# openai/Video-Pre-Training

Measured on AMD Instinct MI355X. Metric: frames/sec (fwd) [+ bc_step.ms_per_step], 2x policy, 128x128x3 seq=128, higher is better.
Workload: dtype bf16; 1 GPU; foundation-model-2x policy forward (IMPALA CNN + 4-layer banded transformer + heads), batch=64 seq=128 uint8 128x128x3 frames per GPU, KV memory carried, random-init weights; global_batch=64, seq_len=128, parallelism=dp1 replicas (no collective in forward; BC step: gradient all-reduce)

## Files before the change

include/vpt_hip.h:

```cpp
#ifndef VPT_HIP_H
#define VPT_HIP_H
#include <stdint.h>

#ifdef __cplusplus
extern "C" {
#endif

const char* vpt_version(void);
#define VPT_HIP_ABI 5
int vpt_abi_version(void);
const char* vpt_operand_format(void);
const char* vpt_last_error(void);

long vpt_conv3x3_packed_elems(int Cout, int Cin);
long vpt_conv3x3_table_floats(int Cout);
long vpt_linear_packed_elems(int N, int K);
long vpt_conv_first_packed_elems(int Cout);
long vpt_conv3d_t5_packed_elems(int O);
int vpt_pack_conv_first(const float* weight, const float* bias, void* wfrag, int Cout, void* stream);
int vpt_pack_conv3d_t5(const float* weight, const float* bias, void* wfrag, float* bias_padded, int O, void* stream);
int vpt_chw_to_blocked(const float* src, float* dst, int64_t rows, int C, int H, int W, void* stream);

enum { VPT_WS_CONV3X3_WGRAD = 1, VPT_WS_CONV_BACKWARD_PREPARE = 2, VPT_WS_LINEAR_SPLITK = 3, VPT_WS_LAYERNORM_BACKWARD = 4, VPT_WS_COLUMN_SUM = 5,
       VPT_WS_ATTENTION_BACKWARD_DKV = 6, VPT_WS_ATTENTION_BACKWARD_DBND = 7, VPT_WS_FRAME_AFFINE_BACKWARD = 8, VPT_WS_CONV_FIRST_BACKWARD = 9 };
// ... 48 lines not shown

int vpt_linear_wgrad(const void* dy, const void* x, float* dw, int M, int N, int K, int ldy, int ldx, int ldw, int accumulate, void* stream);

int vpt_dense_fold_epilogue(const float* part, int splitk, const double* stats, int count, const float* sg, const float* sb, float* out,
                            int M, int N, void* stream);

int vpt_linear_splitk_epilogue(const float* part, int splitk, const float* bias, const float* res, float* out_f32, void* out_bf16,
                               int M, int N, int ldr, int ldc, int ldcb, int relu, const void* mask, int ldm, void* stream);

int vpt_layernorm_linear_forward(const float* x, const float* ln_gain, const float* ln_bias, int relu_in, float* ln_out_f32,
                                 const void* wpk, const float* bias, const float* res, float* out_f32, void* out_bf16,
                                 int M, int N, int K, int ldr, int ldc, int ldcb, int relu, void* stream);

int vpt_layernorm_forward(const float* x, const float* gain, const float* bias, float* out_f32, void* out_bf16,
                          int M, int D, int relu_in, void* stream);

int vpt_masked_attention_forward(const float* qkvr, const float* kmem, const float* vmem, const uint8_t* memvalid,
                                 const float* b_nd, void* out, int B, int t, int heads, int hid, int ld,
                                 int maxlen, int causal, void* stream);

int vpt_kv_memory_update(const float* qkvr, const float* kmem, const float* vmem, float* kout, float* vout,
                         int B, int t, int hid, int ld, int maxlen, void* stream);

int vpt_masked_attention_step(const float* qkvr, const float* kmem, const float* vmem, const uint8_t* state_mask, const uint8_t* first,
                              const float* b_nd, void* out, float* kout, float* vout, uint8_t* mask_out,
                              int B, int heads, int hid, int ld, int maxlen, void* stream);

int vpt_masked_attention_step_inplace(const float* qkvr, float* kmem, float* vmem, uint8_t* state_mask, const uint8_t* first,
                                      const float* b_nd, void* out, int* done_counter, int B, int heads, int hid, int ld, int maxlen, void* stream);

int vpt_act_epilogue(const int64_t* action_buttons, const int64_t* action_camera, const float* logp_buttons, const float* logp_camera,
                     const float* logits, int ld, int value_col, float scale, float shift, int64_t* keep, uint8_t* nan_flag, uint64_t* rng_state,
                     int B, void* stream);

int vpt_log_softmax_forward(const float* logits, float* out, int M, int ld, int col0, int n, float temperature,
                            void* stream);

int vpt_action_head_forward(const float* logits, const uint8_t* mask, const float* noise, const uint64_t* rng_state, uint32_t rng_stream,
                            float* out, int64_t* action, float* action_logp, int M, int ld, int col0, int n, float temperature, void* stream);
int vpt_uniform_noise(const uint64_t* rng_state, uint32_t rng_stream, float* out, int M, int n, void* stream);

int vpt_adam_step(float* param, const float* grad, float* exp_avg, float* exp_avg_sq, uint64_t n, int step,
                  float lr, float beta1, float beta2, float eps, float weight_decay, float grad_scale, void* stream);

int vpt_adam_step_multi(const void* table, int ntensors, int64_t total_blocks, int step, float lr, float beta1, float beta2,
                        float eps, float weight_decay, float grad_scale, const int32_t* skip_flag, void* stream);
// ... 73 lines not shown
```

video-pre-training_amd/_native.py:

```python
import ctypes
import os

_HERE = os.path.dirname(os.path.abspath(__file__))
_LIB_PATH = os.environ.get("VPT_HIP_LIB") or os.path.join(_HERE, "libvpt_hip.so")
_LIB_PATHS = {"bf16": _LIB_PATH, "fp16": os.path.join(_HERE, "libvpt_hip_f16.so")}
_libs = {}

ABI_VERSION = 5

_P = ctypes.c_void_p
_I = ctypes.c_int
_F = ctypes.c_float
_L = ctypes.c_long
_D = ctypes.c_double

SIGNATURES = {
    "vpt_conv_first_forward": [_P, _P, _P, _P, _P, _P, _I, _I, _I, _I, _P],
    "vpt_conv3d_t5_forward": [_P, _P, _P, _P, _P, _I, _I, _I, _I, _I, _P],
    "vpt_pack_conv3x3": [_P, _P, _P, _P, _P, _P, _I, _I, _P],
    "vpt_pack_linear": [_P, _P, _I, _I, _I, _I, _I, _P],
    "vpt_pack_conv_first": [_P, _P, _P, _I, _P],
    "vpt_pack_conv3d_t5": [_P, _P, _P, _P, _I, _P],
    "vpt_chw_to_blocked": [_P, _P, ctypes.c_int64, _I, _I, _I, _P],
    "vpt_conv3x3_forward": [_P, _P, _P, _P, _P, _P, _P, _P, _I, _I, _I, _I, _I, _P],
    "vpt_conv3x3_forward_tiled": [_P, _P, _P, _P, _P, _P, _P, _P, _I, _I, _I, _I, _I, _I, _P],
    "vpt_conv3x3_pool_forward": [_P, _P, _P, _P, _P, _P, _P, _P, _P, _P, _I, _I, _I, _I, _I, _I, _P],
    "vpt_conv3x3_forward_folded": [_P] * 12 + [_I, _I, _I, _I, _I, _P],
    "vpt_channel_stats": [_P, _P, _I, _I, _I, _P],
    "vpt_nfold_coef": [_P] * 12 + [_I, _I, _I, _I, _P],
    "vpt_maxpool_forward": [_P, _P, _P, _P, _I, _I, _I, _I, _P],
    "vpt_frame_affine_forward": [_P, _P, _P, _P, _P, _P, _I, _I, _I, _I, _P],
    "vpt_linear_forward": [_P, _P, _P, _P, _P, _P, _I, _I, _I, _I, _I, _I, _I, _I, _I, _P, _I, _P],
    "vpt_linear_forward_tiled": [_P, _P, _P, _P, _P, _P, _I, _I, _I, _I, _I, _I, _I, _I, _I, _P, _I, _I, _P],
    "vpt_linear_wgrad": [_P, _P, _P, _I, _I, _I, _I, _I, _I, _I, _P],
    "vpt_dense_fold_epilogue": [_P, _I, _P, _I, _P, _P, _P, _I, _I, _P],
    "vpt_linear_splitk_epilogue": [_P, _I, _P, _P, _P, _P, _I, _I, _I, _I, _I, _I, _P, _I, _P],
    "vpt_layernorm_forward": [_P, _P, _P, _P, _P, _I, _I, _I, _P],
    "vpt_masked_attention_forward": [_P, _P, _P, _P, _P, _P, _I, _I, _I, _I, _I, _I, _I, _P],
    "vpt_kv_memory_update": [_P, _P, _P, _P, _P, _I, _I, _I, _I, _I, _P],
    "vpt_log_softmax_forward": [_P, _P, _I, _I, _I, _I, _F, _P],
    "vpt_action_head_forward": [_P, _P, _P, _P, ctypes.c_uint32, _P, _P, _P, _I, _I, _I, _I, _F, _P],
    "vpt_uniform_noise": [_P, ctypes.c_uint32, _P, _I, _I, _P],
    "vpt_conv_backward_prepare": [_P] * 14 + [_I, _I, _I, _I, _I, _P],
    "vpt_conv3x3_dgrad": [_P, _P, _P, _P, _P, _P, _I, _I, _I, _I, _I, _P],
    "vpt_conv3x3_pool_argmax_forward": [_P, _P, _P, _P, _P, _P, _P, _P, _P, _I, _I, _I, _I, _I, _I, _P],
    "vpt_conv_backward_prepare_pooled": [_P] * 15 + [_I, _I, _I, _I, _I, _P],
    "vpt_conv3x3_dgrad_gated": [_P, _P, _P, _P, _P, _I, _P, _P, _I, _I, _I, _I, _I, _P],
    "vpt_conv_backward_reduce": [_P] * 10 + [_I, _I, _I, _I, _I, _P],
    "vpt_conv_first_backward": [_P, _P, _P, _P, _P, _P, _I, _I, _I, _I, _P],
    "vpt_conv_first_backward_nfold": [_P, _P, _P, _P, _P, _P, _P, _P, _P, _I, _I, _I, _I, _P],
    "vpt_conv3x3_wgrad": [_P, _P, _P, _P, _I, _I, _I, _I, _I, _P],
    "vpt_conv3x3_wgrad_scratch_floats": [_I, _I, _I],
    "vpt_camera_discretize": [_P, _P, _L, _D, _D, _D, _I, _P],
    "vpt_camera_undiscretize": [_P, _P, _L, _D, _D, _D, _I, _P],
    "vpt_action_from_factored": [_P, _P, _P, _P, _L, _I, _P],
    "vpt_action_to_factored": [_P, _P, _P, _P, _L, _I, _P],
    "vpt_maxpool_backward": [_P, _P, _P, _P, _I, _I, _I, _I, _P],
    "vpt_frame_affine_backward": [_P, _P, _P, _P, _P, _P, _P, _P, _P, _P, _I, _I, _I, _I, _I, _P],
    "vpt_bc_nll_backward": [_P, _P, _P, _P, _P, _I, _I, _I, _I, _F, _P],
    "vpt_heads_logprob_backward": [_P, _P, _P, _P, _P, _P, _P, _P, _I, _I, _I, _I, _F, _F, _P],
    "vpt_layernorm_backward": [_P, _P, _P, _P, _P, _P, _P, _P, _I, _I, _I, _P],
    "vpt_gate_cast": [_P, _P, _P, _I, _I, _I, _I, _I, _P],
# ... 73 lines not shown
```

video-pre-training_amd/csrc/vpt_capi.hip:

```cpp
#include "../../include/vpt_hip.h"
#include "vpt_kernels.h"
#include "vpt_common.h"
#include <stdio.h>
#include <math.h>

static thread_local char g_err[256] = "ok";

static int fail(int code, const char* what) {
  snprintf(g_err, sizeof(g_err), "%s (code %d, hip: %s)", what, code, hipGetErrorString(hipPeekAtLastError()));
  return code;
}
#define CHECK_LAUNCH(expr, name) do { int rc_ = (expr); if (rc_ != 0) return fail(rc_, name); return 0; } while (0)

__global__ __launch_bounds__(256) void vpt_poison_lds_kernel(int words, unsigned pattern) {
  extern __shared__ unsigned poison_lds_[];
  volatile unsigned* l = poison_lds_;
  for (int i = threadIdx.x; i < words; i += 256) l[i] = pattern;
  __syncthreads();
  for (int k = 0; k < 16; ++k) __builtin_amdgcn_s_sleep(127);
}

extern "C" {

const char* vpt_version(void) { return "vpt_hip 0.5 gfx950"; }
// ... 368 lines not shown
  a.A = nullptr; a.wpk = nullptr; a.bias = bias; a.res = res; a.out_f32 = out_f32; a.out_bf16 = (vpt_op16*)out_bf16;
  a.M = M; a.N = N; a.K = 0; a.lda = 0; a.ldr = ldr; a.ldc = ldc; a.ldcb = ldcb; a.relu = relu; a.splitk = splitk; a.atomic_out = 0;
  a.mask = (const vpt_op16*)mask; a.ldm = ldm;
  CHECK_LAUNCH(vpt_splitk_epilogue_launch(part, splitk, &a, (hipStream_t)stream), "vpt_linear_splitk_epilogue");
}

int vpt_layernorm_forward(const float* x, const float* gain, const float* bias, float* out_f32, void* out_bf16,
                          int M, int D, int relu_in, void* stream) {
  VptLayerNormArgs a = {};
  a.x = x; a.gain = gain; a.bias = bias; a.out_f32 = out_f32; a.out_bf16 = (vpt_op16*)out_bf16;
  a.M = M; a.D = D; a.relu_in = relu_in;
  CHECK_LAUNCH(vpt_layernorm_launch(&a, (hipStream_t)stream), "vpt_layernorm_forward");
}

int vpt_masked_attention_forward(const float* qkvr, const float* kmem, const float* vmem, const uint8_t* memvalid,
                                 const float* b_nd, void* out, int B, int t, int heads, int hid, int ld,
                                 int maxlen, int causal, void* stream) {
  VptAttnArgs a = {};
  a.qkvr = qkvr; a.kmem = kmem; a.vmem = vmem; a.memvalid = memvalid; a.b_nd = b_nd; a.out = (vpt_op16*)out;
  a.B = B; a.t = t; a.heads = heads; a.hid = hid; a.ld = ld; a.maxlen = maxlen; a.causal = causal;
  CHECK_LAUNCH(vpt_attn_launch(&a, (hipStream_t)stream), "vpt_masked_attention_forward");
}

int vpt_masked_attention_step(const float* qkvr, const float* kmem, const float* vmem, const uint8_t* state_mask, const uint8_t* first,
                              const float* b_nd, void* out, float* kout, float* vout, uint8_t* mask_out,
                              int B, int heads, int hid, int ld, int maxlen, void* stream) {
  VptAttnArgs a = {};
  a.qkvr = qkvr; a.kmem = kmem; a.vmem = vmem; a.memvalid = nullptr; a.b_nd = b_nd; a.out = (vpt_op16*)out;
  a.B = B; a.t = 1; a.heads = heads; a.hid = hid; a.ld = ld; a.maxlen = maxlen; a.causal = 1;
  CHECK_LAUNCH(vpt_attn_step_launch(&a, state_mask, first, mask_out, kout, vout, nullptr, (hipStream_t)stream), "vpt_masked_attention_step");
}

int vpt_masked_attention_step_inplace(const float* qkvr, float* kmem, float* vmem, uint8_t* state_mask, const uint8_t* first,
                                      const float* b_nd, void* out, int* done_counter, int B, int heads, int hid, int ld, int maxlen, void* stream) {
  if (!done_counter) return fail(-1, "vpt_masked_attention_step_inplace: done_counter ([B] ints, zero before the first launch) is required");
  VptAttnArgs a = {};
  a.qkvr = qkvr; a.kmem = kmem; a.vmem = vmem; a.memvalid = nullptr; a.b_nd = b_nd; a.out = (vpt_op16*)out;
  a.B = B; a.t = 1; a.heads = heads; a.hid = hid; a.ld = ld; a.maxlen = maxlen; a.causal = 1;
  CHECK_LAUNCH(vpt_attn_step_launch(&a, state_mask, first, state_mask, kmem, vmem, done_counter, (hipStream_t)stream), "vpt_masked_attention_step_inplace");
}

int vpt_act_epilogue(const int64_t* action_buttons, const int64_t* action_camera, const float* logp_buttons, const float* logp_camera,
                     const float* logits, int ld, int value_col, float scale, float shift, int64_t* keep, uint8_t* nan_flag, uint64_t* rng_state,
                     int B, void* stream) {
  CHECK_LAUNCH(vpt_act_epilogue_launch(action_buttons, action_camera, logp_buttons, logp_camera, logits, ld, value_col, scale, shift, keep, nan_flag,
                                       rng_state, B, (hipStream_t)stream), "vpt_act_epilogue");
// ... 149 lines not shown
```

video-pre-training_amd/csrc/vpt_kernels.h:

```cpp
#pragma once
#include <hip/hip_runtime.h>
#include <stdint.h>

#ifdef VPT_OPERAND_F16
typedef _Float16 vpt_op16;
#else
typedef __bf16 vpt_op16;
#endif

struct VptConv3x3Args {
  const vpt_op16* x;
  const vpt_op16* wpk;
  const float* edge_sa;
  const float* edge_sg;
  const double* stats_in;
  const vpt_op16* res;
  vpt_op16* y;
  double* stats_out;
  int frames, H, W, Cin, Cout, CoutPad, NT;
  double inv_count_in;
  int tiling;
  int ablate;
  long long* trace;
  const float* kk_frame;
// ... 364 lines not shown
int vpt_colsum_launch(const VptColsumArgs* a, hipStream_t s);
int vpt_clip_launch(const VptClipArgs* a, hipStream_t s);
int vpt_attn_step_launch(const VptAttnArgs* a, const uint8_t* state_mask, const uint8_t* first, uint8_t* mask_out, float* kout, float* vout, int* done, hipStream_t s);
int vpt_act_epilogue_launch(const int64_t* act_b, const int64_t* act_c, const float* lp_b, const float* lp_c, const float* logits, int ld, int vcol,
                            float scale, float shift, int64_t* keep, uint8_t* nan_flag, uint64_t* rng_state, int B, hipStream_t s);
int vpt_uniform_noise_launch(const uint64_t* rng_state, uint32_t rng_stream, float* out, int M, int n, hipStream_t s);
int vpt_attn_bwd_launch(const VptAttnBwdArgs* a, hipStream_t s);
long vpt_attn_bwd_dkv_floats(int B, int t, int hid);
long vpt_attn_bwd_dbnd_floats(int B, int t, int heads, int maxlen);
long vpt_colsum_partial_floats(int M, int N);
long vpt_slab_sum_scratch_floats(int rows, int cols);
int vpt_slab_sum_launch(const float* slab, int rows, int cols, long ld, float* out_a, int split, float* out_b, int accumulate, float* scratch, hipStream_t s);
int vpt_conv3x3_launch(const VptConv3x3Args* a, hipStream_t s);
int vpt_pool_seam_launch(const VptPoolSeamArgs* a, hipStream_t s);
int vpt_channel_stats_launch(const VptChannelStatsArgs* a, hipStream_t s);
int vpt_nfold_coef_launch(const VptNfoldCoefArgs* a, hipStream_t s);
int vpt_conv_first_launch(const VptConvFirstArgs* a, hipStream_t s);
int vpt_conv3d_launch(const VptConv3dArgs* a, hipStream_t s);
int vpt_pool_launch(const VptPoolArgs* a, hipStream_t s);
int vpt_affine_launch(const VptAffineArgs* a, hipStream_t s);
int vpt_gemm_launch(const VptGemmArgs* a, hipStream_t s);
int vpt_layernorm_launch(const VptLayerNormArgs* a, hipStream_t s);
int vpt_attn_launch(const VptAttnArgs* a, hipStream_t s);
int vpt_kv_update_launch(const VptKvUpdateArgs* a, hipStream_t s);
int vpt_logsoftmax_launch(const VptLogSoftmaxArgs* a, hipStream_t s);
}
```

video-pre-training_amd/csrc/vpt_transformer.hip:

```cpp
#include "vpt_common.h"
#include "vpt_kernels.h"

__global__ __launch_bounds__(256) void vpt_layernorm_kernel(VptLayerNormArgs a) {
  const int lane = threadIdx.x & 63;
  const int row = blockIdx.x * 4 + (threadIdx.x >> 6);
  if (row >= a.M) return;
  const float* x = a.x + (size_t)row * a.D;
  const int n4 = a.D >> 2;
  float s = 0.f;
  for (int i = lane; i < n4; i += 64) {
    f32x4 v = *(const f32x4*)(x + 4 * i);
    if (a.relu_in) { v.x = fmaxf(v.x, 0.f); v.y = fmaxf(v.y, 0.f); v.z = fmaxf(v.z, 0.f); v.w = fmaxf(v.w, 0.f); }
    s += (v.x + v.y) + (v.z + v.w);
  }
  const float mean = wave_sum(s) / (float)a.D;
  float ss = 0.f;
  for (int i = lane; i < n4; i += 64) {
    f32x4 v = *(const f32x4*)(x + 4 * i);
    if (a.relu_in) { v.x = fmaxf(v.x, 0.f); v.y = fmaxf(v.y, 0.f); v.z = fmaxf(v.z, 0.f); v.w = fmaxf(v.w, 0.f); }
    const float d0 = v.x - mean, d1 = v.y - mean, d2 = v.z - mean, d3 = v.w - mean;
    ss += (d0 * d0 + d1 * d1) + (d2 * d2 + d3 * d3);
  }
  const float rstd = rsqrtf(wave_sum(ss) / (float)a.D + VPT_NORM_EPS);
  for (int i = lane; i < n4; i += 64) {
// ... 10 lines not shown
      u32x2 p = {pack_op16x2(y.x, y.y), pack_op16x2(y.z, y.w)};
      *(u32x2*)(a.out_bf16 + (size_t)row * a.D + 4 * i) = p;
    }
  }
}

extern "C" int vpt_layernorm_launch(const VptLayerNormArgs* a, hipStream_t stream) {
  if (a->M <= 0 || (a->D & 3)) return -1;
  hipLaunchKernelGGL(vpt_layernorm_kernel, dim3((a->M + 3) >> 2), dim3(256), 0, stream, *a);
  return hipGetLastError() == hipSuccess ? 0 : -3;
}

#define ATT_DH 128
#define ATT_QT 32
#define ATT_NK 160
#define ATT_RS (ATT_DH + 4)
#define ATT_SS 164
#define ATT_S_OFF 0
#define ATT_R_OFF (ATT_S_OFF + ATT_QT * ATT_SS)
#define ATT_B_OFF (ATT_R_OFF + ATT_QT * 10)
#define ATT_SC_OFF (ATT_B_OFF + 10 * 129)
#define ATT_PT_OFF ((ATT_SC_OFF + ATT_QT + 3) & ~3)
#define ATT_FLOATS (ATT_PT_OFF + 4 * 16 * 64)

__global__ __launch_bounds__(256) void vpt_attn_kernel(VptAttnArgs a) {
  extern __shared__ __attribute__((aligned(16))) float sm[];
  float* Ss = sm + ATT_S_OFF;
  float* Rs = sm + ATT_R_OFF;
  float* Bs = sm + ATT_B_OFF;
  float* Sc = sm + ATT_SC_OFF;

  const int tid = threadIdx.x, lane = tid & 63, w = __builtin_amdgcn_readfirstlane(tid >> 6);
  const int b = blockIdx.y / a.heads, h = blockIdx.y - b * a.heads;
  const int q0 = blockIdx.x * ATT_QT;
  const int maxlen = a.maxlen, t = a.t, hid = a.hid;
  const size_t tok0 = (size_t)b * t;
  const int jbase = a.causal ? q0 + 1 : 0;

  for (int idx = tid; idx < ATT_QT * 10; idx += 256) {
    const int r = idx / 10, n = idx - r * 10;
    Rs[idx] = (a.causal && q0 + r < t) ? a.qkvr[(tok0 + q0 + r) * a.ld + 3 * hid + h * 10 + n] : 0.f;
  }
  for (int idx = tid; idx < 10 * maxlen; idx += 256) Bs[idx] = a.b_nd[idx];
  __syncthreads();

  const int l31 = lane & 31, hi = lane >> 5;
  auto kv_row = [&](int j, int which) -> const float* {
    if (j < maxlen) return (which == 1 ? a.kmem : a.vmem) + ((size_t)b * maxlen + j) * hid + h * ATT_DH;
    if (j - maxlen < t) return a.qkvr + (tok0 + j - maxlen) * a.ld + which * hid + h * ATT_DH;
    return nullptr;
  };
  {
    f32x16 acc, acc4;
#pragma unroll
    for (int r = 0; r < 16; ++r) { acc[r] = 0.f; acc4[r] = 0.f; }
    const f32x4 z4 = {0.f, 0.f, 0.f, 0.f};
    const float* qa = (q0 + l31 < t) ? a.qkvr + (tok0 + q0 + l31) * a.ld + h * ATT_DH + 4 * hi : nullptr;
    const float* kr = kv_row(jbase + w * 32 + l31, 1);
    const float* kr4 = kv_row(jbase + 128 + l31, 1);
    const float* kb = kr ? kr + 4 * hi : nullptr;
    const float* kb4 = kr4 ? kr4 + 4 * hi : nullptr;
#pragma unroll 8
    for (int g = 0; g < 16; ++g) {
      const f32x4 q4 = qa ? *(const f32x4*)(qa + 8 * g) : z4, k4 = kb ? *(const f32x4*)(kb + 8 * g) : z4;
      acc = __builtin_amdgcn_mfma_f32_32x32x2f32(q4.x, k4.x, acc, 0, 0, 0);
      acc = __builtin_amdgcn_mfma_f32_32x32x2f32(q4.y, k4.y, acc, 0, 0, 0);
      acc = __builtin_amdgcn_mfma_f32_32x32x2f32(q4.z, k4.z, acc, 0, 0, 0);
      acc = __builtin_amdgcn_mfma_f32_32x32x2f32(q4.w, k4.w, acc, 0, 0, 0);
    }
#pragma unroll
    for (int g4 = 0; g4 < 4; ++g4) {
      const int g = 4 * w + g4;
      const f32x4 q4 = qa ? *(const f32x4*)(qa + 8 * g) : z4, k4 = kb4 ? *(const f32x4*)(kb4 + 8 * g) : z4;
      acc4 = __builtin_amdgcn_mfma_f32_32x32x2f32(q4.x, k4.x, acc4, 0, 0, 0);
      acc4 = __builtin_amdgcn_mfma_f32_32x32x2f32(q4.y, k4.y, acc4, 0, 0, 0);
      acc4 = __builtin_amdgcn_mfma_f32_32x32x2f32(q4.z, k4.z, acc4, 0, 0, 0);
      acc4 = __builtin_amdgcn_mfma_f32_32x32x2f32(q4.w, k4.w, acc4, 0, 0, 0);
    }
    float* Pt = sm + ATT_PT_OFF;
#pragma unroll
    for (int r = 0; r < 16; ++r) Pt[(w * 16 + r) * 64 + lane] = acc4[r];
    __syncthreads();
    auto finish = [&](int kk, int r, float dot) {
      const int qi = (r & 3) + 8 * (r >> 2) + 4 * hi;
      const bool qvalid = (q0 + qi) < t;
      const int off = maxlen - 1 + qi - kk;
      const int j = jbase + kk;
      bool vis = a.causal ? (qvalid && off >= 0 && off < maxlen) : (qvalid && kk < t);
      if (vis && a.causal && j < maxlen) vis = a.memvalid[(size_t)b * maxlen + j] != 0;
      float sc = -3.0e38f;
      if (vis) {
        float rb = 0.f;
        if (a.causal) {
#pragma unroll
          for (int n = 0; n < 10; ++n) rb = fmaf(Rs[qi * 10 + n], Bs[n * maxlen + off], rb);
        }
        sc = dot * (1.0f / ATT_DH) + rb;
      }
      Ss[qi * ATT_SS + kk] = sc;
    };
#pragma unroll
    for (int r = 0; r < 16; ++r) finish(w * 32 + l31, r, acc[r]);
#pragma unroll
    for (int r4 = 0; r4 < 4; ++r4) {
      const int r = 4 * w + r4;
      const float dot = (Pt[(0 * 16 + r) * 64 + lane] + Pt[(1 * 16 + r) * 64 + lane]) + (Pt[(2 * 16 + r) * 64 + lane] + Pt[(3 * 16 + r) * 64 + lane]);
      finish(128 + l31, r, dot);
    }
  }
  __syncthreads();
  for (int r = w * 8; r < w * 8 + 8; ++r) {
    float* srow = Ss + r * ATT_SS;
    const float s0 = srow[lane], s1 = srow[lane + 64], s2 = (lane + 128 < ATT_NK) ? srow[lane + 128] : -3.0e38f;
    const float m = wave_max(fmaxf(s0, fmaxf(s1, s2)));
    const float e0 = (s0 > -1.0e38f) ? expf(s0 - m) : 0.f;
    const float e1 = (s1 > -1.0e38f) ? expf(s1 - m) : 0.f;
    const float e2 = (s2 > -1.0e38f) ? expf(s2 - m) : 0.f;
    const float tot = wave_sum(e0 + e1 + e2);
    srow[lane] = e0;
    srow[lane + 64] = e1;
    if (lane + 128 < ATT_NK) srow[lane + 128] = e2;
    if (lane == 0) Sc[r] = (tot > 0.f) ? 1.0f / tot : 0.f;
  }
  __syncthreads();

  {
    f32x16 o;
#pragma unroll
    for (int r = 0; r < 16; ++r) o[r] = 0.f;
    const float* pa = Ss + l31 * ATT_SS + 4 * hi;
    const int dcol = w * 32 + l31;
#pragma unroll 4
    for (int g = 0; g < ATT_NK / 8; ++g) {
      const f32x4 p4 = *(const f32x4*)(pa + 8 * g);
      float v[4];
#pragma unroll
      for (int e = 0; e < 4; ++e) {
        const float* r0 = kv_row(jbase + 8 * g + e, 2);
        const float* r1 = kv_row(jbase + 8 * g + 4 + e, 2);
        const float* rr = hi ? r1 : r0;
        v[e] = rr ? rr[dcol] : 0.f;
      }
      o = __builtin_amdgcn_mfma_f32_32x32x2f32(p4.x, v[0], o, 0, 0, 0);
      o = __builtin_amdgcn_mfma_f32_32x32x2f32(p4.y, v[1], o, 0, 0, 0);
      o = __builtin_amdgcn_mfma_f32_32x32x2f32(p4.z, v[2], o, 0, 0, 0);
      o = __builtin_amdgcn_mfma_f32_32x32x2f32(p4.w, v[3], o, 0, 0, 0);
    }
#pragma unroll
    for (int r = 0; r < 16; ++r) {
      const int qi = (r & 3) + 8 * (r >> 2) + 4 * hi;
      if (q0 + qi < t) a.out[(tok0 + q0 + qi) * hid + h * ATT_DH + w * 32 + l31] = (vpt_op16)(o[r] * Sc[qi]);
    }
  }
}

extern "C" int vpt_attn_launch(const VptAttnArgs* a, hipStream_t stream) {
  if (a->hid != a->heads * ATT_DH) return -1;
  if (a->causal ? (a->maxlen < 1 || a->maxlen > 129) : (a->maxlen != 0 || a->t > ATT_NK)) return -1;
  static unsigned long long optin_done = 0;
  const size_t lds = ATT_FLOATS * sizeof(float);
  if (!vpt_lds_optin((const void*)vpt_attn_kernel, (int)lds, &optin_done)) return -4;
  dim3 grid((a->t + ATT_QT - 1) / ATT_QT, a->B * a->heads);
  hipLaunchKernelGGL(vpt_attn_kernel, grid, dim3(256), lds, stream, *a);
  return hipGetLastError() == hipSuccess ? 0 : -3;
}

struct VptAttnStepExtra {
  const uint8_t* state_mask;
  const uint8_t* first;
  uint8_t* mask_out;
  float* kout;
  float* vout;
  int* done;
};

__global__ __launch_bounds__(256) void vpt_attn_step_kernel(VptAttnArgs a, VptAttnStepExtra x) {
  __shared__ float sc_[128], red_[8], part_[128];
  __shared__ int last_;
  const int tid = threadIdx.x, lane = tid & 63, w = tid >> 6;
  const int b = blockIdx.x / a.heads, h = blockIdx.x - b * a.heads;
  const int maxlen = a.maxlen, hid = a.hid;
  const float* qrow = a.qkvr + (size_t)b * a.ld;
  auto kv_row = [&](int j, int which) -> const float* {
    if (j < maxlen) return (which == 1 ? a.kmem : a.vmem) + ((size_t)b * maxlen + j) * hid + h * ATT_DH;
    return qrow + which * hid + h * ATT_DH;
  };
// ... 94 lines not shown
  const int h4 = a.hid >> 2;
  const int c4 = (int)(idx % h4);
  const size_t rs = idx / h4;
  const int s = (int)(rs % a.maxlen);
  const int b = (int)(rs / a.maxlen);
  const int src = s + a.t;
  const float* mem = which ? a.vmem : a.kmem;
  float* out = which ? a.vout : a.kout;
  f32x4 v;
  if (src < a.maxlen) v = *(const f32x4*)(mem + ((size_t)b * a.maxlen + src) * a.hid + c4 * 4);
  else v = *(const f32x4*)(a.qkvr + ((size_t)b * a.t + (src - a.maxlen)) * a.ld + (which ? 2 : 1) * a.hid + c4 * 4);
  *(f32x4*)(out + ((size_t)b * a.maxlen + s) * a.hid + c4 * 4) = v;
}

extern "C" int vpt_kv_update_launch(const VptKvUpdateArgs* a, hipStream_t stream) {
  if (a->B <= 0 || (a->hid & 3)) return -1;
  const size_t n4 = (size_t)a->B * a->maxlen * (a->hid >> 2);
  dim3 grid((unsigned)((n4 + 255) / 256), 2);
  hipLaunchKernelGGL(vpt_kv_update_kernel, grid, dim3(256), 0, stream, *a);
  return hipGetLastError() == hipSuccess ? 0 : -3;
}

#define LSM_CAP 9
template <int NW>
__global__ __launch_bounds__(64 * NW) void vpt_logsoftmax_kernel(VptLogSoftmaxArgs a) {
  constexpr int NT = 64 * NW;
  __shared__ float red[3 * NW];
  __shared__ int redi[NW];
  const int row = blockIdx.x, tid = threadIdx.x, lane = tid & 63, w = tid >> 6;
  const float* z = a.logits + (size_t)row * a.ld + a.col0;
  const uint8_t* mk = a.mask ? a.mask + (size_t)row * a.n : nullptr;
  const float T = a.temperature;
#define SCALED(i_) ((mk && !mk[i_]) ? -100.0f : z[i_] / T)
  float c[LSM_CAP];
  float m = -3.0e38f;
#pragma unroll
  for (int k = 0; k < LSM_CAP; ++k) {
    const int i = tid + NT * k;
    c[k] = (i < a.n) ? SCALED(i) : -3.0e38f;
    m = fmaxf(m, c[k]);
  }
  for (int i = tid + NT * LSM_CAP; i < a.n; i += NT) m = fmaxf(m, SCALED(i));
  m = wave_max(m);
  if (lane == 0) red[w] = m;
  __syncthreads();
  m = red[0];
#pragma unroll
  for (int k = 1; k < NW; ++k) m = fmaxf(m, red[k]);
  float s = 0.f;
#pragma unroll
  for (int k = 0; k < LSM_CAP; ++k) s += (tid + NT * k < a.n) ? expf(c[k] - m) : 0.f;
  for (int i = tid + NT * LSM_CAP; i < a.n; i += NT) s += expf(SCALED(i) - m);
  s = wave_sum(s);
  if (lane == 0) red[NW + w] = s;
  __syncthreads();
  float tot = 0.f;
#pragma unroll
  for (int k = 0; k < NW; ++k) tot += red[NW + k];
  const float lse = m + logf(tot);
  float* o = a.out + (size_t)row * a.n;
  const float* u = a.noise ? a.noise + (size_t)row * a.n : nullptr;
  const bool gen = !u && a.rng_state != nullptr;
  uint64_t seed = 0, rstep = 0;
  if (gen) { seed = a.rng_state[0]; rstep = a.rng_state[1]; }
  float best = -3.0e38f;
  int besti = 0x7fffffff;
  auto emit = [&](int i, float sc_) __attribute__((always_inline)) {
    const float lp = sc_ - lse;
    o[i] = lp;
    if (a.action) {
      float sc = lp;
      if (u || gen) {
        float ui = u ? u[i] : vpt_philox_uniform(seed, rstep, a.rng_stream, (uint32_t)row, (uint32_t)i);
        if (ui == 1.0f) ui = 0.999f;
        sc = lp - logf(-logf(ui));
      }
      if (sc > best) { best = sc; besti = i; }
    }
  };
#pragma unroll
  for (int k = 0; k < LSM_CAP; ++k)
    if (tid + NT * k < a.n) emit(tid + NT * k, c[k]);
  for (int i = tid + NT * LSM_CAP; i < a.n; i += NT) emit(i, SCALED(i));
  if (a.action) {
#pragma unroll
    for (int off = 32; off > 0; off >>= 1) {
      const float ob = __shfl_xor(best, off, 64);
      const int oi = __shfl_xor(besti, off, 64);
      if (ob > best || (ob == best && oi < besti)) { best = ob; besti = oi; }
    }
    if (lane == 0) { red[2 * NW + w] = best; redi[w] = besti; }
    __syncthreads();
    if (tid == 0) {
      for (int k = 1; k < NW; ++k)
        if (red[2 * NW + k] > best || (red[2 * NW + k] == best && redi[k] < besti)) { best = red[2 * NW + k]; besti = redi[k]; }
      a.action[row] = besti;
      if (a.action_logp) a.action_logp[row] = ((mk && !mk[besti]) ? -100.0f : z[besti] / T) - lse;
    }
  }
#undef SCALED
}

extern "C" int vpt_logsoftmax_launch(const VptLogSoftmaxArgs* a, hipStream_t stream) {
  if (a->M <= 0 || a->n <= 0) return -1;
  if (a->M < 64 && a->n > 1024) hipLaunchKernelGGL((vpt_logsoftmax_kernel<16>), dim3(a->M), dim3(1024), 0, stream, *a);
  else hipLaunchKernelGGL((vpt_logsoftmax_kernel<4>), dim3(a->M), dim3(256), 0, stream, *a);
  return hipGetLastError() == hipSuccess ? 0 : -3;
}

__global__ void vpt_act_epilogue_kernel(const int64_t* act_b, const int64_t* act_c, const float* lp_b, const float* lp_c, const float* logits, int ld,
                                        int vcol, float scale, float shift, int64_t* keep, uint8_t* nan_flag, uint64_t* rng_state, int B) {
  const int b = threadIdx.x;
  bool bad = false;
  if (b < B) {
    const float lp = lp_b[b] + lp_c[b];
    const float v = logits[(size_t)b * ld + vcol];
    const float vd = fmaf(v, scale, shift);
    bad = lp != lp;
    keep[4 * b + 0] = act_b[b];
    keep[4 * b + 1] = act_c[b];
    keep[4 * b + 2] = (int64_t)(uint64_t)__builtin_bit_cast(uint32_t, lp);
    keep[4 * b + 3] = (int64_t)((uint64_t)__builtin_bit_cast(uint32_t, vd) | ((uint64_t)__builtin_bit_cast(uint32_t, v) << 32));
  }
  const unsigned long long any = __ballot(bad);
  if (threadIdx.x == 0) {
    *nan_flag = any ? 1 : 0;
    if (rng_state) rng_state[1] += 1;
  }
}
// ... 25 lines not shown
```

video-pre-training_amd/engine.py:

```python
import os
from typing import Dict, List, Optional

import torch

from . import ops, packing

DENSE_SPLITK = int(os.environ.get("VPT_DENSE_SPLITK", "32"))


def config_from_policy_kwargs(policy_kwargs: dict, pi_head_kwargs: Optional[dict] = None) -> dict:
    pk = policy_kwargs
    width = pk.get("impala_width", 1)
    chans = [int(width * c) for c in pk.get("impala_chans", (16, 32, 32))]
    cfg = dict(
        chans=chans,
        hidsize=pk.get("hidsize", 512),
        heads=pk.get("attention_heads", 8),
        n_layers=pk.get("n_recurrence_layers", 1),
        maxlen=pk.get("attention_memory_size", 2048) - (pk.get("timesteps") or 0),
        causal=pk.get("attention_mask_style", "clipped_causal") == "clipped_causal",
        pointwise_ratio=pk.get("pointwise_ratio", 4),
        use_pre_lstm_ln=pk.get("use_pre_lstm_ln", True),
        temperature=float((pi_head_kwargs or {}).get("temperature", 1.0)),
        img_shape=list(pk.get("img_shape") or [128, 128, 3]),
# ... 391 lines not shown
    @torch.no_grad()
    def forward(self, img_u8: torch.Tensor, first: torch.Tensor, state_in: List, mask: Optional[dict] = None,
                sample: Optional[str] = None, inplace_state: bool = False, act_tail: Optional[tuple] = None):
        if not self.packed:
            raise RuntimeError("PolicyEngine.pack(state_dict) must be called before forward")
        cfg, w = self.cfg, self.w
        bsz, t = img_u8.shape[:2]
        hid, heads, maxlen = cfg["hidsize"], cfg["heads"], cfg["maxlen"]
        frames = img_u8.reshape(bsz * t, *img_u8.shape[2:]).contiguous()
        frames_ready = None
        if self.step_overlap and frames.data_ptr() != img_u8.data_ptr() and not torch.cuda.is_current_stream_capturing():
            frames_ready = torch.cuda.Event()
            frames_ready.record(torch.cuda.current_stream())
        tiling = "latency" if (t == 1 and bsz <= ops.LN_LINEAR_MAX_ROWS) else "throughput"
        x = self._img_process(frames, tiling=tiling, frames_ready=frames_ready)
        if cfg["use_pre_lstm_ln"]:
            x, _ = ops.layernorm(x, w["prelstm.g"], w["prelstm.b"], out_f32=True, out_bf16=False, dtype=self.dtype)

        step = t == 1 and maxlen <= ops.ATTENTION_STEP_MAXLEN
        if inplace_state and not step:
            raise ValueError("inplace_state is the acting step's option (T = 1)")
        if step:
            first8 = first[:, 0].contiguous().view(torch.uint8)
        else:
            not_first = ~first[:, 0].reshape(bsz, 1, 1)
        state_out = []
        for l in range(cfg["n_layers"]):
            p = f"net.recurrent_layer.blocks.{l}."
            state_mask, (kmem, vmem) = state_in[l]
            if state_mask is None:
                state_mask = torch.zeros(bsz, 1, maxlen, dtype=torch.bool, device=x.device)
            x1, qkvr, _ = self._ln_linear(x, w[p + "ln1.g"], w[p + "ln1.b"], w[p + "qkvr.w"], self.n_qkvr, bias=w[p + "qkvr.b"], ln_out_f32=True, tiling=tiling)
            if step:
                if inplace_state and not (kmem.is_contiguous() and vmem.is_contiguous()):
                    raise ValueError("inplace_state needs contiguous state tensors (a .contiguous() copy would receive the update instead of the state)")
                done = None
                if inplace_state:
                    if not state_mask.is_contiguous():
                        raise ValueError("inplace_state needs contiguous state masks")
                    if self._attn_done is None or self._attn_done.device != x.device:
                        self._attn_done = torch.zeros(64, dtype=torch.int32, device=x.device)
                    done = self._attn_done
                att, kout, vout, m8 = ops.masked_attention_step(qkvr, kmem.contiguous(), vmem.contiguous(), state_mask.reshape(bsz, maxlen).contiguous(), first8,
                                                               w[p + "b_nd"], bsz, heads, hid, dtype=self.dtype, inplace=inplace_state, done=done)
                new_mask = state_mask if inplace_state else m8.view(torch.bool).view(bsz, 1, maxlen)
            else:
                memvalid = (state_mask & not_first).reshape(bsz, maxlen).to(torch.uint8).contiguous()
                att = ops.masked_attention(qkvr, kmem.contiguous(), vmem.contiguous(), memvalid, w[p + "b_nd"], bsz, t, heads, hid, dtype=self.dtype)
                kout, vout = ops.kv_memory_update(qkvr, kmem.contiguous(), vmem.contiguous(), bsz, t, hid)
                new_mask = torch.cat([state_mask[:, :, t:] & not_first,
                                      torch.ones(bsz, 1, min(t, maxlen), dtype=torch.bool, device=x.device)], dim=-1)
            x2, _ = ops.linear(att, w[p + "proj.w"], hid, bias=w[p + "proj.b"], res=x1, tiling=tiling)
            _, _, h2 = self._ln_linear(x2, w[p + "ln2.g"], w[p + "ln2.b"], w[p + "mlp0.w"], hid * cfg["pointwise_ratio"], relu=True,
                                       out_f32=False, out_bf16=True, tiling=tiling)
            x, _ = ops.linear(h2, w[p + "mlp1.w"], hid, bias=w[p + "mlp1.b"], res=x2, tiling=tiling)
            state_out.append((new_mask, (kout, vout)))

        _, y, _ = self._ln_linear(x, w["last.g"], w["last.b"], w["last.w"], hid, relu=True, relu_in=True, tiling=tiling)
        nb, nc = self.n_buttons, self.n_camera
        latent, logits, _ = self._ln_linear(y, w["final.g"], w["final.b"], w["heads.w"], nb + nc + 1, bias=w["heads.b"], ln_out_f32=True, tiling=tiling)
        temp = cfg["temperature"]
        out = dict(latent=latent.view(bsz, t, hid), state_out=state_out)
        tail = act_tail is not None and sample is not None and t == 1
        rng = self.rng_state(x.device) if sample == "stochastic" else None
        heads_out = action_heads(logits, (("buttons", 0, 1, nb), ("camera", nb, 1, nc)), bsz, t, temp, mask, sample, keep_head_logps=tail, rng_state=rng)
        out.update(heads_out)
        if tail:
            lps = out.pop("_head_logps")
            keep, flag = ops.act_epilogue(out["action"]["buttons"].view(-1), out["action"]["camera"].view(-1), lps["buttons"].reshape(-1),
                                          lps["camera"].reshape(-1), logits, nb + nc, act_tail[0], act_tail[1], rng_state=rng)
            out["_keep"], out["nan_flag"] = keep, flag
            out.update(unpack_act_tail(keep, bsz))
        else:
            out["vpred"] = logits[:, nb + nc:nb + nc + 1].reshape(bsz, t, 1).clone()
# ... 130 lines not shown
```

video-pre-training_amd/ops.py:

```python
import ctypes
import os

import torch

from . import _native
from ._native import ptr


def _stream():
    return ctypes.c_void_p(torch.cuda.current_stream().cuda_stream)


class KernelTimer:

    def __init__(self):
        self.enabled = False
        self.records = []

    def reset(self):
        self.records = []

    def summary(self):
        torch.cuda.synchronize()
        out = {}
# ... 429 lines not shown
          batch, t, heads, hid, qkv.shape[1], 0, 0, _stream(), fmt=fmt)
    return out


def masked_attention(qkvr, kmem, vmem, memvalid, b_nd, batch, t, heads, hid, dtype=torch.bfloat16):
    _chk(qkvr, torch.float32, "qkvr"); _chk(kmem, torch.float32, "kmem"); _chk(vmem, torch.float32, "vmem")
    _chk(memvalid, torch.uint8, "memvalid"); _chk(b_nd, torch.float32, "b_nd")
    maxlen = kmem.shape[1]
    dt, fmt = _fmt(dtype=dtype)
    out = torch.empty(batch * t, hid, dtype=dt, device=qkvr.device)
    _call("vpt_masked_attention_forward", dict(flops=4.0 * batch * t * (t + maxlen) * hid), ptr(qkvr), ptr(kmem), ptr(vmem), ptr(memvalid), ptr(b_nd), ptr(out),
                 batch, t, heads, hid, qkvr.shape[1], maxlen, 1, _stream(), fmt=fmt)
    return out


def kv_memory_update(qkvr, kmem, vmem, batch, t, hid):
    _chk(qkvr, torch.float32, "qkvr"); _chk(kmem, torch.float32, "kmem"); _chk(vmem, torch.float32, "vmem")
    kout, vout = torch.empty_like(kmem), torch.empty_like(vmem)
    _call("vpt_kv_memory_update", dict(bytes=16.0 * batch * kmem.shape[1] * hid), ptr(qkvr), ptr(kmem), ptr(vmem), ptr(kout), ptr(vout),
                 batch, t, hid, qkvr.shape[1], kmem.shape[1], _stream())
    return kout, vout


ATTENTION_STEP_MAXLEN = 128


def masked_attention_step(qkvr, kmem, vmem, state_mask, first, b_nd, batch, heads, hid, dtype=torch.bfloat16, inplace=False, done=None):
    _chk(qkvr, torch.float32, "qkvr"); _chk(kmem, torch.float32, "kmem"); _chk(vmem, torch.float32, "vmem"); _chk(b_nd, torch.float32, "b_nd")
    if state_mask.dtype == torch.bool:
        state_mask = state_mask.view(torch.uint8)
    if first.dtype == torch.bool:
        first = first.view(torch.uint8)
    _chk(state_mask, torch.uint8, "state_mask"); _chk(first, torch.uint8, "first")
    maxlen = kmem.shape[1]
    if qkvr.shape[0] != batch or maxlen > ATTENTION_STEP_MAXLEN or tuple(state_mask.shape) != (batch, maxlen) or first.numel() != batch:
        raise ValueError(f"masked_attention_step: one token per sequence, maxlen <= {ATTENTION_STEP_MAXLEN}, state_mask [batch, maxlen], first [batch] "
                         f"(got {qkvr.shape[0]} rows for batch {batch}, maxlen {maxlen}, mask {tuple(state_mask.shape)})")
    dt, fmt = _fmt(dtype=dtype)
    out = torch.empty(batch, hid, dtype=dt, device=qkvr.device)
    meta = dict(flops=4.0 * batch * maxlen * hid, bytes=16.0 * batch * maxlen * hid)
    if done is not None:
        if not inplace:
            raise ValueError("masked_attention_step: `done` is the in-place variant's counter")
        if done.dtype != torch.int32 or done.numel() < batch or not done.is_contiguous():
            raise ValueError("masked_attention_step: done must be a contiguous int32 tensor of at least `batch` zeros")
        _call("vpt_masked_attention_step_inplace", meta, ptr(qkvr), ptr(kmem), ptr(vmem), ptr(state_mask), ptr(first), ptr(b_nd), ptr(out), ptr(done),
# ... 383 lines not shown
```

Before: 78420 frames/s.

## Fuse masked attention with KV memory update and mask construction

```diff
diff --git a/include/vpt_hip.h b/include/vpt_hip.h
--- a/include/vpt_hip.h
+++ b/include/vpt_hip.h
@@ -94,6 +94,10 @@
 int vpt_kv_memory_update(const float* qkvr, const float* kmem, const float* vmem, float* kout, float* vout,
                          int B, int t, int hid, int ld, int maxlen, void* stream);
 
+int vpt_masked_attention_fused(const float* qkvr, const float* kmem, const float* vmem, const uint8_t* state_mask, const uint8_t* first,
+                               int first_ld, const float* b_nd, void* out, float* kout, float* vout, uint8_t* mask_out,
+                               int B, int t, int heads, int hid, int ld, int maxlen, void* stream);
+
 int vpt_masked_attention_step(const float* qkvr, const float* kmem, const float* vmem, const uint8_t* state_mask, const uint8_t* first,
                               const float* b_nd, void* out, float* kout, float* vout, uint8_t* mask_out,
                               int B, int heads, int hid, int ld, int maxlen, void* stream);
diff --git a/video-pre-training_amd/_native.py b/video-pre-training_amd/_native.py
--- a/video-pre-training_amd/_native.py
+++ b/video-pre-training_amd/_native.py
@@ -38,6 +38,7 @@
     "vpt_layernorm_forward": [_P, _P, _P, _P, _P, _I, _I, _I, _P],
     "vpt_masked_attention_forward": [_P, _P, _P, _P, _P, _P, _I, _I, _I, _I, _I, _I, _I, _P],
     "vpt_kv_memory_update": [_P, _P, _P, _P, _P, _I, _I, _I, _I, _I, _P],
+    "vpt_masked_attention_fused": [_P, _P, _P, _P, _P, _I, _P, _P, _P, _P, _P, _I, _I, _I, _I, _I, _I, _P],
     "vpt_log_softmax_forward": [_P, _P, _I, _I, _I, _I, _F, _P],
     "vpt_action_head_forward": [_P, _P, _P, _P, ctypes.c_uint32, _P, _P, _P, _I, _I, _I, _I, _F, _P],
     "vpt_uniform_noise": [_P, ctypes.c_uint32, _P, _I, _I, _P],
diff --git a/video-pre-training_amd/csrc/vpt_capi.hip b/video-pre-training_amd/csrc/vpt_capi.hip
--- a/video-pre-training_amd/csrc/vpt_capi.hip
+++ b/video-pre-training_amd/csrc/vpt_capi.hip
@@ -414,6 +414,15 @@
   CHECK_LAUNCH(vpt_attn_launch(&a, (hipStream_t)stream), "vpt_masked_attention_forward");
 }
 
+int vpt_masked_attention_fused(const float* qkvr, const float* kmem, const float* vmem, const uint8_t* state_mask, const uint8_t* first,
+                               int first_ld, const float* b_nd, void* out, float* kout, float* vout, uint8_t* mask_out,
+                               int B, int t, int heads, int hid, int ld, int maxlen, void* stream) {
+  VptAttnArgs a = {};
+  a.qkvr = qkvr; a.kmem = kmem; a.vmem = vmem; a.memvalid = nullptr; a.b_nd = b_nd; a.out = (vpt_op16*)out;
+  a.B = B; a.t = t; a.heads = heads; a.hid = hid; a.ld = ld; a.maxlen = maxlen; a.causal = 1;
+  CHECK_LAUNCH(vpt_attn_fused_launch(&a, state_mask, first, first_ld, mask_out, kout, vout, (hipStream_t)stream), "vpt_masked_attention_fused");
+}
+
 int vpt_masked_attention_step(const float* qkvr, const float* kmem, const float* vmem, const uint8_t* state_mask, const uint8_t* first,
                               const float* b_nd, void* out, float* kout, float* vout, uint8_t* mask_out,
                               int B, int heads, int hid, int ld, int maxlen, void* stream) {
diff --git a/video-pre-training_amd/csrc/vpt_kernels.h b/video-pre-training_amd/csrc/vpt_kernels.h
--- a/video-pre-training_amd/csrc/vpt_kernels.h
+++ b/video-pre-training_amd/csrc/vpt_kernels.h
@@ -410,6 +410,8 @@
 int vpt_gemm_launch(const VptGemmArgs* a, hipStream_t s);
 int vpt_layernorm_launch(const VptLayerNormArgs* a, hipStream_t s);
 int vpt_attn_launch(const VptAttnArgs* a, hipStream_t s);
+int vpt_attn_fused_launch(const VptAttnArgs* a, const uint8_t* state_mask, const uint8_t* first, int first_ld, uint8_t* mask_out,
+                          float* kout, float* vout, hipStream_t s);
 int vpt_kv_update_launch(const VptKvUpdateArgs* a, hipStream_t s);
 int vpt_logsoftmax_launch(const VptLogSoftmaxArgs* a, hipStream_t s);
 }
diff --git a/video-pre-training_amd/csrc/vpt_transformer.hip b/video-pre-training_amd/csrc/vpt_transformer.hip
--- a/video-pre-training_amd/csrc/vpt_transformer.hip
+++ b/video-pre-training_amd/csrc/vpt_transformer.hip
@@ -56,20 +56,43 @@
 #define ATT_SC_OFF (ATT_B_OFF + 10 * 129)
 #define ATT_PT_OFF ((ATT_SC_OFF + ATT_QT + 3) & ~3)
 #define ATT_FLOATS (ATT_PT_OFF + 4 * 16 * 64)
-
-__global__ __launch_bounds__(256) void vpt_attn_kernel(VptAttnArgs a) {
-  extern __shared__ __attribute__((aligned(16))) float sm[];
+#define ATT_FUSED_FLOATS (ATT_SC_OFF + ATT_QT)
+
+struct VptAttnFusedExtra {
+  const uint8_t* state_mask;
+  const uint8_t* first;
+  int first_ld;
+  uint8_t* mask_out;
+  float* kout;
+  float* vout;
+};
+
+template <bool FUSED>
+__device__ __forceinline__ void attn_tile(const VptAttnArgs& a, const VptAttnFusedExtra& x, float* sm, const int qt, const int bh) {
   float* Ss = sm + ATT_S_OFF;
   float* Rs = sm + ATT_R_OFF;
   float* Bs = sm + ATT_B_OFF;
   float* Sc = sm + ATT_SC_OFF;
 
   const int tid = threadIdx.x, lane = tid & 63, w = __builtin_amdgcn_readfirstlane(tid >> 6);
-  const int b = blockIdx.y / a.heads, h = blockIdx.y - b * a.heads;
-  const int q0 = blockIdx.x * ATT_QT;
+  const int b = bh / a.heads, h = bh - b * a.heads;
+  const int q0 = qt * ATT_QT;
   const int maxlen = a.maxlen, t = a.t, hid = a.hid;
   const size_t tok0 = (size_t)b * t;
   const int jbase = a.causal ? q0 + 1 : 0;
+  bool fst0 = false;
+  int own_lo = 0, own_hi = 0;
+  if constexpr (FUSED) {
+    fst0 = x.first[(size_t)b * x.first_ld] != 0;
+    own_lo = max(t, qt == 0 ? 0 : maxlen + q0) - jbase;
+    own_hi = min(t + maxlen, maxlen + q0 + ATT_QT) - jbase;
+    if (qt == 0 && h == 0) {
+      for (int s = tid; s < maxlen; s += 256) {
+        const int src = s + t;
+        x.mask_out[(size_t)b * maxlen + s] = (src < maxlen) ? ((x.state_mask[(size_t)b * maxlen + src] != 0 && !fst0) ? 1 : 0) : 1;
+      }
+    }
+  }
 
   for (int idx = tid; idx < ATT_QT * 10; idx += 256) {
     const int r = idx / 10, n = idx - r * 10;
@@ -111,17 +134,31 @@
       acc4 = __builtin_amdgcn_mfma_f32_32x32x2f32(q4.z, k4.z, acc4, 0, 0, 0);
       acc4 = __builtin_amdgcn_mfma_f32_32x32x2f32(q4.w, k4.w, acc4, 0, 0, 0);
     }
-    float* Pt = sm + ATT_PT_OFF;
+    float* Pt = sm + (FUSED ? ATT_S_OFF : ATT_PT_OFF);
 #pragma unroll
     for (int r = 0; r < 16; ++r) Pt[(w * 16 + r) * 64 + lane] = acc4[r];
     __syncthreads();
+    auto tile4_dot = [&](int r4) {
+      const int r = 4 * w + r4;
+      return (Pt[(0 * 16 + r) * 64 + lane] + Pt[(1 * 16 + r) * 64 + lane]) + (Pt[(2 * 16 + r) * 64 + lane] + Pt[(3 * 16 + r) * 64 + lane]);
+    };
+    float dot4[4];
+    if constexpr (FUSED) {
+#pragma unroll
+      for (int r4 = 0; r4 < 4; ++r4) dot4[r4] = tile4_dot(r4);
+      __syncthreads();
+    }
     auto finish = [&](int kk, int r, float dot) {
       const int qi = (r & 3) + 8 * (r >> 2) + 4 * hi;
       const bool qvalid = (q0 + qi) < t;
       const int off = maxlen - 1 + qi - kk;
       const int j = jbase + kk;
       bool vis = a.causal ? (qvalid && off >= 0 && off < maxlen) : (qvalid && kk < t);
-      if (vis && a.causal && j < maxlen) vis = a.memvalid[(size_t)b * maxlen + j] != 0;
+      if constexpr (FUSED) {
+        if (vis && j < maxlen) vis = x.state_mask[(size_t)b * maxlen + j] != 0 && !fst0;
+      } else {
+        if (vis && a.causal && j < maxlen) vis = a.memvalid[(size_t)b * maxlen + j] != 0;
+      }
       float sc = -3.0e38f;
       if (vis) {
         float rb = 0.f;
@@ -136,11 +173,7 @@
 #pragma unroll
     for (int r = 0; r < 16; ++r) finish(w * 32 + l31, r, acc[r]);
 #pragma unroll
-    for (int r4 = 0; r4 < 4; ++r4) {
-      const int r = 4 * w + r4;
-      const float dot = (Pt[(0 * 16 + r) * 64 + lane] + Pt[(1 * 16 + r) * 64 + lane]) + (Pt[(2 * 16 + r) * 64 + lane] + Pt[(3 * 16 + r) * 64 + lane]);
-      finish(128 + l31, r, dot);
-    }
+    for (int r4 = 0; r4 < 4; ++r4) finish(128 + l31, 4 * w + r4, FUSED ? dot4[r4] : tile4_dot(r4));
   }
   __syncthreads();
   for (int r = w * 8; r < w * 8 + 8; ++r) {
@@ -186,6 +219,42 @@
       if (q0 + qi < t) a.out[(tok0 + q0 + qi) * hid + h * ATT_DH + w * 32 + l31] = (vpt_op16)(o[r] * Sc[qi]);
     }
   }
+  if constexpr (FUSED) {
+    const int total = 2 * (own_hi - own_lo) * (ATT_DH / 4);
+    for (int base = 0; base < total; base += 8 * 256) {
+      f32x4 v[8];
+#pragma unroll
+      for (int u = 0; u < 8; ++u) {
+        const int idx = base + u * 256 + tid;
+        if (idx < total) {
+          const int which = idx >= total / 2, rem = idx - which * (total / 2);
+          v[u] = *(const f32x4*)(kv_row(jbase + own_lo + (rem >> 5), 1 + which) + 4 * (rem & 31));
+        }
+      }
+#pragma unroll
+      for (int u = 0; u < 8; ++u) {
+        const int idx = base + u * 256 + tid;
+        if (idx < total) {
+          const int which = idx >= total / 2, rem = idx - which * (total / 2);
+          float* dst = (which ? x.vout : x.kout) + ((size_t)b * maxlen + (jbase + own_lo + (rem >> 5) - t)) * hid + h * ATT_DH;
+          *(f32x4*)(dst + 4 * (rem & 31)) = v[u];
+        }
+      }
+    }
+  }
+}
+
+__global__ __launch_bounds__(256) void vpt_attn_kernel(VptAttnArgs a) {
+  extern __shared__ __attribute__((aligned(16))) float sm[];
+  attn_tile<false>(a, VptAttnFusedExtra{}, sm, blockIdx.x, blockIdx.y);
+}
+
+__global__ __launch_bounds__(256) void vpt_attn_fused_kernel(VptAttnArgs a, VptAttnFusedExtra x) {
+  extern __shared__ __attribute__((aligned(16))) float sm[];
+  const int nt = (a.t + ATT_QT - 1) / ATT_QT;
+  const int L = xcd_remap(blockIdx.x, gridDim.x);
+  const int bh = L / nt;
+  attn_tile<true>(a, x, sm, L - bh * nt, bh);
 }
 
 extern "C" int vpt_attn_launch(const VptAttnArgs* a, hipStream_t stream) {
@@ -196,6 +265,30 @@
   if (!vpt_lds_optin((const void*)vpt_attn_kernel, (int)lds, &optin_done)) return -4;
   dim3 grid((a->t + ATT_QT - 1) / ATT_QT, a->B * a->heads);
   hipLaunchKernelGGL(vpt_attn_kernel, grid, dim3(256), lds, stream, *a);
+  return hipGetLastError() == hipSuccess ? 0 : -3;
+}
+
+static bool vpt_ranges_overlap(const void* p, const void* q, size_t bytes) {
+  const char *a = (const char*)p, *b = (const char*)q;
+  return a < b + bytes && b < a + bytes;
+}
+
+extern "C" int vpt_attn_fused_launch(const VptAttnArgs* a, const uint8_t* state_mask, const uint8_t* first, int first_ld, uint8_t* mask_out,
+                                     float* kout, float* vout, hipStream_t stream) {
+  if (a->hid != a->heads * ATT_DH || !a->causal || a->maxlen < 1 || a->maxlen > 129 || a->t < 1 || a->B < 1) return -1;
+  if (!a->kmem || !a->vmem || !state_mask || !first || first_ld < 1 || !mask_out || !kout || !vout) return -1;
+  const size_t mem_bytes = (size_t)a->B * a->maxlen * a->hid * sizeof(float);
+  if (vpt_ranges_overlap(kout, a->kmem, mem_bytes) || vpt_ranges_overlap(kout, a->vmem, mem_bytes) ||
+      vpt_ranges_overlap(vout, a->kmem, mem_bytes) || vpt_ranges_overlap(vout, a->vmem, mem_bytes) ||
+      vpt_ranges_overlap(kout, vout, mem_bytes) || vpt_ranges_overlap(mask_out, state_mask, (size_t)a->B * a->maxlen)) return -1;
+  static unsigned long long optin_done = 0;
+  const size_t lds = ATT_FUSED_FLOATS * sizeof(float);
+  if (!vpt_lds_optin((const void*)vpt_attn_fused_kernel, (int)lds, &optin_done)) return -4;
+  VptAttnFusedExtra x;
+  x.state_mask = state_mask; x.first = first; x.first_ld = first_ld; x.mask_out = mask_out; x.kout = kout; x.vout = vout;
+  const long nwg = (long)((a->t + ATT_QT - 1) / ATT_QT) * a->B * a->heads;
+  if (nwg > 0x7fffffffL) return -1;
+  hipLaunchKernelGGL(vpt_attn_fused_kernel, dim3((unsigned)nwg), dim3(256), lds, stream, *a, x);
   return hipGetLastError() == hipSuccess ? 0 : -3;
 }
 
@@ -336,9 +429,11 @@
 }
 
 #define LSM_CAP 9
-template <int NW>
+#define LSM_ROW_LDS_MAX 16000
+template <int NW, int CAP, bool ROW_LDS = false>
 __global__ __launch_bounds__(64 * NW) void vpt_logsoftmax_kernel(VptLogSoftmaxArgs a) {
   constexpr int NT = 64 * NW;
+  extern __shared__ float rowv[];
   __shared__ float red[3 * NW];
   __shared__ int redi[NW];
   const int row = blockIdx.x, tid = threadIdx.x, lane = tid & 63, w = tid >> 6;
@@ -346,15 +441,37 @@
   const uint8_t* mk = a.mask ? a.mask + (size_t)row * a.n : nullptr;
   const float T = a.temperature;
 #define SCALED(i_) ((mk && !mk[i_]) ? -100.0f : z[i_] / T)
-  float c[LSM_CAP];
+  float c[CAP];
   float m = -3.0e38f;
-#pragma unroll
-  for (int k = 0; k < LSM_CAP; ++k) {
-    const int i = tid + NT * k;
-    c[k] = (i < a.n) ? SCALED(i) : -3.0e38f;
-    m = fmaxf(m, c[k]);
-  }
-  for (int i = tid + NT * LSM_CAP; i < a.n; i += NT) m = fmaxf(m, SCALED(i));
+  if constexpr (ROW_LDS) {
+    for (int i0 = tid; i0 < a.n; i0 += 8 * NT) {
+      float zv[8];
+      uint8_t mv[8];
+#pragma unroll
+      for (int u = 0; u < 8; ++u) {
+        const int i = min(i0 + u * NT, a.n - 1);
+        zv[u] = z[i];
+        mv[u] = mk ? mk[i] : (uint8_t)1;
+      }
+#pragma unroll
+      for (int u = 0; u < 8; ++u) {
+        const int i = i0 + u * NT;
+        if (i < a.n) {
+          const float v = mv[u] ? zv[u] / T : -100.0f;
+          rowv[i] = v;
+          m = fmaxf(m, v);
+        }
+      }
+    }
+  } else {
+#pragma unroll
+    for (int k = 0; k < CAP; ++k) {
+      const int i = tid + NT * k;
+      c[k] = (i < a.n) ? SCALED(i) : -3.0e38f;
+      m = fmaxf(m, c[k]);
+    }
+    for (int i = tid + NT * CAP; i < a.n; i += NT) m = fmaxf(m, SCALED(i));
+  }
   m = wave_max(m);
   if (lane == 0) red[w] = m;
   __syncthreads();
@@ -362,9 +479,13 @@
 #pragma unroll
   for (int k = 1; k < NW; ++k) m = fmaxf(m, red[k]);
   float s = 0.f;
-#pragma unroll
-  for (int k = 0; k < LSM_CAP; ++k) s += (tid + NT * k < a.n) ? expf(c[k] - m) : 0.f;
-  for (int i = tid + NT * LSM_CAP; i < a.n; i += NT) s += expf(SCALED(i) - m);
+  if constexpr (ROW_LDS) {
+    for (int i = tid; i < a.n; i += NT) s += expf(rowv[i] - m);
+  } else {
+#pragma unroll
+    for (int k = 0; k < CAP; ++k) s += (tid + NT * k < a.n) ? expf(c[k] - m) : 0.f;
+    for (int i = tid + NT * CAP; i < a.n; i += NT) s += expf(SCALED(i) - m);
+  }
   s = wave_sum(s);
   if (lane == 0) red[NW + w] = s;
   __syncthreads();
@@ -392,10 +513,14 @@
       if (sc > best) { best = sc; besti = i; }
     }
   };
-#pragma unroll
-  for (int k = 0; k < LSM_CAP; ++k)
-    if (tid + NT * k < a.n) emit(tid + NT * k, c[k]);
-  for (int i = tid + NT * LSM_CAP; i < a.n; i += NT) emit(i, SCALED(i));
+  if constexpr (ROW_LDS) {
+    for (int i = tid; i < a.n; i += NT) emit(i, rowv[i]);
+  } else {
+#pragma unroll
+    for (int k = 0; k < CAP; ++k)
+      if (tid + NT * k < a.n) emit(tid + NT * k, c[k]);
+    for (int i = tid + NT * CAP; i < a.n; i += NT) emit(i, SCALED(i));
+  }
   if (a.action) {
 #pragma unroll
     for (int off = 32; off > 0; off >>= 1) {
@@ -417,8 +542,10 @@
 
 extern "C" int vpt_logsoftmax_launch(const VptLogSoftmaxArgs* a, hipStream_t stream) {
   if (a->M <= 0 || a->n <= 0) return -1;
-  if (a->M < 64 && a->n > 1024) hipLaunchKernelGGL((vpt_logsoftmax_kernel<16>), dim3(a->M), dim3(1024), 0, stream, *a);
-  else hipLaunchKernelGGL((vpt_logsoftmax_kernel<4>), dim3(a->M), dim3(256), 0, stream, *a);
+  if (a->M < 64 && a->n > 1024) hipLaunchKernelGGL((vpt_logsoftmax_kernel<16, LSM_CAP>), dim3(a->M), dim3(1024), 0, stream, *a);
+  else if (a->n > 4 * 64 * LSM_CAP && a->n <= LSM_ROW_LDS_MAX)
+    hipLaunchKernelGGL((vpt_logsoftmax_kernel<4, 1, true>), dim3(a->M), dim3(256), (size_t)a->n * sizeof(float), stream, *a);
+  else hipLaunchKernelGGL((vpt_logsoftmax_kernel<4, LSM_CAP>), dim3(a->M), dim3(256), 0, stream, *a);
   return hipGetLastError() == hipSuccess ? 0 : -3;
 }
 
diff --git a/video-pre-training_amd/engine.py b/video-pre-training_amd/engine.py
--- a/video-pre-training_amd/engine.py
+++ b/video-pre-training_amd/engine.py
@@ -437,8 +437,6 @@
             raise ValueError("inplace_state is the acting step's option (T = 1)")
         if step:
             first8 = first[:, 0].contiguous().view(torch.uint8)
-        else:
-            not_first = ~first[:, 0].reshape(bsz, 1, 1)
         state_out = []
         for l in range(cfg["n_layers"]):
             p = f"net.recurrent_layer.blocks.{l}."
@@ -460,11 +458,9 @@
                                                                w[p + "b_nd"], bsz, heads, hid, dtype=self.dtype, inplace=inplace_state, done=done)
                 new_mask = state_mask if inplace_state else m8.view(torch.bool).view(bsz, 1, maxlen)
             else:
-                memvalid = (state_mask & not_first).reshape(bsz, maxlen).to(torch.uint8).contiguous()
-                att = ops.masked_attention(qkvr, kmem.contiguous(), vmem.contiguous(), memvalid, w[p + "b_nd"], bsz, t, heads, hid, dtype=self.dtype)
-                kout, vout = ops.kv_memory_update(qkvr, kmem.contiguous(), vmem.contiguous(), bsz, t, hid)
-                new_mask = torch.cat([state_mask[:, :, t:] & not_first,
-                                      torch.ones(bsz, 1, min(t, maxlen), dtype=torch.bool, device=x.device)], dim=-1)
+                att, kout, vout, m8 = ops.masked_attention_fused(qkvr, kmem.contiguous(), vmem.contiguous(), state_mask.reshape(bsz, maxlen).contiguous(), first,
+                                                                 w[p + "b_nd"], bsz, t, heads, hid, dtype=self.dtype)
+                new_mask = m8.view(torch.bool).view(bsz, 1, maxlen)
             x2, _ = ops.linear(att, w[p + "proj.w"], hid, bias=w[p + "proj.b"], res=x1, tiling=tiling)
             _, _, h2 = self._ln_linear(x2, w[p + "ln2.g"], w[p + "ln2.b"], w[p + "mlp0.w"], hid * cfg["pointwise_ratio"], relu=True,
                                        out_f32=False, out_bf16=True, tiling=tiling)
diff --git a/video-pre-training_amd/ops.py b/video-pre-training_amd/ops.py
--- a/video-pre-training_amd/ops.py
+++ b/video-pre-training_amd/ops.py
@@ -475,6 +475,29 @@
     return kout, vout
 
 
+def masked_attention_fused(qkvr, kmem, vmem, state_mask, first, b_nd, batch, t, heads, hid, dtype=torch.bfloat16):
+    _chk(qkvr, torch.float32, "qkvr"); _chk(kmem, torch.float32, "kmem"); _chk(vmem, torch.float32, "vmem"); _chk(b_nd, torch.float32, "b_nd")
+    if state_mask.dtype == torch.bool:
+        state_mask = state_mask.view(torch.uint8)
+    if first.dtype == torch.bool:
+        first = first.view(torch.uint8)
+    _chk(state_mask, torch.uint8, "state_mask")
+    if first.dtype != torch.uint8 or not first.is_cuda:
+        raise TypeError("masked_attention_fused: first must be a bool / uint8 CUDA tensor")
+    maxlen = kmem.shape[1]
+    if qkvr.shape[0] != batch * t or tuple(state_mask.shape) != (batch, maxlen) or not state_mask.is_contiguous() or first.shape[0] != batch:
+        raise ValueError(f"masked_attention_fused: qkvr [batch * t, ld], state_mask contiguous [batch, maxlen], first [batch, ...] "
+                         f"(got {tuple(qkvr.shape)} for batch {batch}, t {t}; mask {tuple(state_mask.shape)}; first {tuple(first.shape)})")
+    dt, fmt = _fmt(dtype=dtype)
+    out = torch.empty(batch * t, hid, dtype=dt, device=qkvr.device)
+    kout, vout = torch.empty_like(kmem), torch.empty_like(vmem)
+    mout = torch.empty_like(state_mask)
+    _call("vpt_masked_attention_fused", dict(flops=4.0 * batch * t * (t + maxlen) * hid, bytes=16.0 * batch * maxlen * hid),
+          ptr(qkvr), ptr(kmem), ptr(vmem), ptr(state_mask), ptr(first), first.stride(0), ptr(b_nd), ptr(out), ptr(kout), ptr(vout), ptr(mout),
+          batch, t, heads, hid, qkvr.shape[1], maxlen, _stream(), fmt=fmt)
+    return out, kout, vout, mout
+
+
 ATTENTION_STEP_MAXLEN = 128
 
 
```

Result: no change. 78920 frames/s, median of 6 (+0.6%).
